# TCLResearchEurope/ptdeco

Measured on AMD Instinct MI355X. Metric: layers decomposed/sec (incl. covariance+SVD), higher is better.
Workload: dtype f64

## Files before the change

### ptdeco_amd/csrc/eigh_tridiag.hip

```cpp
#include <algorithm>
#include <atomic>
#include <cmath>
#include <cstdlib>
#include <cstring>
#include <functional>
#include <mutex>
#include <vector>

#include <hip/hip_ext.h>

#include "common.h"
#include "kernels.h"

namespace ptd {

int gemm_f64(const double* A, int64_t sam, int64_t sak, const double* B, int64_t sbk, int64_t sbn, double* C,
             int64_t ldc, int64_t M, int64_t N, int64_t K, double alpha, bool beta1, int ksplit, hipStream_t st);
int gemm_f64_pair(const double* A, const double* B, const double* A2, const double* B2, int64_t sam, int64_t sak,
                  int64_t sbk, int64_t sbn, double* C, int64_t ldc, int64_t M, int64_t N, int64_t K, double alpha,
                  double* row0_out, hipStream_t st, int batch = 1, int64_t bstride_elems = 0);
int gemm_f64_slabs(const double* A, int64_t sam, int64_t sak, const double* B, int64_t sbk, int64_t sbn, double* C,
                   int64_t ldc, int64_t slab, int64_t M, int64_t N, int64_t K, double alpha, int ksplit, int* nslabs,
                   bool lower_only, hipStream_t st);

// ... 146 lines not shown
        cs->alpha = colbuf[j + 1] - delta * vprev[j + 1];
      }
    }
  }
}

constexpr int TR = 64, TC = 256, TQ = TC / TR;

struct SymPart {
  double* rowpart;
  double* colpart;
  int64_t ldp;
  int nI;
  int enabled;
};

__device__ __forceinline__ double transpose_reduce16(double (&p)[16], int lane) {
  {
    const bool hi = lane & 32;
#pragma unroll
    for (int t = 0; t < 8; ++t) {
      const double send = hi ? p[t] : p[t + 8];
      const double keep = hi ? p[t + 8] : p[t];
      p[t] = keep + __shfl_xor(send, 32);
    }
  }
  {
    const bool hi = lane & 16;
#pragma unroll
    for (int t = 0; t < 4; ++t) {
      const double send = hi ? p[t] : p[t + 4];
      const double keep = hi ? p[t + 4] : p[t];
      p[t] = keep + __shfl_xor(send, 16);
    }
  }
  {
    const bool hi = lane & 8;
#pragma unroll
    for (int t = 0; t < 2; ++t) {
      const double send = hi ? p[t] : p[t + 2];
      const double keep = hi ? p[t + 2] : p[t];
      p[t] = keep + __shfl_xor(send, 8);
    }
  }
  {
    const bool hi = lane & 4;
    const double send = hi ? p[0] : p[1];
    const double keep = hi ? p[1] : p[0];
    p[0] = keep + __shfl_xor(send, 4);
  }
  p[0] += __shfl_xor(p[0], 2);
  p[0] += __shfl_xor(p[0], 1);
  return p[0];
}

template <bool GEN>
__device__ __forceinline__ void symv2_tile_body(const double2 (&a0)[16], const double2 (&a1)[16], const double2 xa,
                                                const double2 xb, const double* __restrict__ xs, int rbase, int nclamp,
                                                int cA, int cB, double (&p)[16], double (&acc)[4]) {
#pragma unroll
  for (int t = 0; t < 16; ++t) {
    const double xr = xs[t];
    double r0 = a0[t].x, r1 = a0[t].y, r2 = a1[t].x, r3 = a1[t].y;
    double c0 = r0, c1 = r1, c2 = r2, c3 = r3;
    if (GEN) {
      const int R = min(rbase + t, nclamp);
      r0 = (cA <= R) ? r0 : 0.0;     c0 = (cA < R) ? c0 : 0.0;
      r1 = (cA + 1 <= R) ? r1 : 0.0; c1 = (cA + 1 < R) ? c1 : 0.0;
      r2 = (cB <= R) ? r2 : 0.0;     c2 = (cB < R) ? c2 : 0.0;
      r3 = (cB + 1 <= R) ? r3 : 0.0; c3 = (cB + 1 < R) ? c3 : 0.0;
    }
    p[t] = (r0 * xa.x + r1 * xa.y) + (r2 * xb.x + r3 * xb.y);
    acc[0] += c0 * xr; acc[1] += c1 * xr; acc[2] += c2 * xr; acc[3] += c3 * xr;
  }
}

#ifdef PTD_RES_PROF
__device__ int symv_dbg;
extern "C" void ptd_debug_symv(int v) { (void)hipMemcpyToSymbol(HIP_SYMBOL(symv_dbg), &v, sizeof(int)); }
#define SYMV_DBG(BIT) (symv_dbg & (BIT))
#else
#define SYMV_DBG(BIT) false
#endif
__global__ __launch_bounds__(256) void sytrd_symv2_kernel(const double* __restrict__ A, int64_t ld, int n, int j, int i,
                                                          const double* __restrict__ colbuf,
                                                          const double* __restrict__ Vp,
                                                          const double* __restrict__ Wp, int64_t ldv,
                                                          const double* __restrict__ wraw_prev,
                                                          const double* __restrict__ partial2, int nparts2,
                                                          const double* __restrict__ taus, SymPart sp, int ntiles,
                                                          int nextra, double* __restrict__ qv,
                                                          double* __restrict__ cb, double* __restrict__ px2,
                                                          ColState* __restrict__ cs, size_t bstride) {
  const size_t boff_ = (size_t)blockIdx.y * bstride;
  PTD_BATCH(A); PTD_BATCH(colbuf); PTD_BATCH(Vp); PTD_BATCH(Wp); PTD_BATCH(wraw_prev); PTD_BATCH(partial2);
  PTD_BATCH(taus); PTD_BATCH(sp.rowpart); PTD_BATCH(sp.colpart); PTD_BATCH(qv); PTD_BATCH(cb); PTD_BATCH(px2);
  PTD_BATCH(cs);
  __shared__ __attribute__((aligned(16))) double xs[TR];
  __shared__ __attribute__((aligned(16))) double colred[4][TC];
  __shared__ double part[4][SROWS];
  const int tid = threadIdx.x, lane = tid & 63, wid = tid >> 6;
  const int b = blockIdx.x;
  const double* vprev = Vp + (int64_t)max(i - 1, 0) * ldv;
  if (SYMV_DBG(1)) return;
  if (b < ntiles) {
    const int g0 = (j + 1) / TC;
    int u = (int)((sqrtf(2.f * (float)b + 1.f) - 1.f) * 0.5f);
    while (TQ / 2 * u * (u + 1) > b) --u;
    while (TQ / 2 * (u + 1) * (u + 2) <= b) ++u;
    const int rem = b - TQ / 2 * u * (u + 1);
    const int I = TQ * (g0 + u) + rem / (u + 1), J = g0 + rem % (u + 1);
    const int R0 = I * TR, C0 = J * TC;
    if (R0 + TR - 1 < j + 1 || R0 >= n) return;
    const int cA = C0 + 2 * lane, cB = cA + 128;
    const int rbase = R0 + 16 * wid;
    double2 a0[16], a1[16];
    const bool liveA = (C0 + 127 >= j + 1) && (C0 <= R0 + TR - 1) && (cA + 1 >= j + 1);
    const bool liveB = (C0 + 255 >= j + 1) && (C0 + 128 <= R0 + TR - 1) && (cB + 1 >= j + 1);
    if (C0 + TC - 1 > R0) {
#pragma unroll
      for (int t = 0; t < 16; ++t) {
        const int rr = min(rbase + t, n - 1);
        const double* rowp = A + (int64_t)rr * ld;
        a0[t] = (liveA && cA <= rr) ? *reinterpret_cast<const double2*>(rowp + cA) : double2{0.0, 0.0};
        a1[t] = (liveB && cB <= rr) ? *reinterpret_cast<const double2*>(rowp + cB) : double2{0.0, 0.0};
      }
    } else {
#pragma unroll
      for (int t = 0; t < 16; ++t) {
        const double* rowp = A + (int64_t)min(rbase + t, n - 1) * ld;
        a0[t] = liveA ? *reinterpret_cast<const double2*>(rowp + cA) : double2{0.0, 0.0};
        a1[t] = liveB ? *reinterpret_cast<const double2*>(rowp + cB) : double2{0.0, 0.0};
      }
    }
    if (SYMV_DBG(2)) {
      double sink = 0.0;
#pragma unroll
      for (int t = 0; t < 16; ++t) sink += a0[t].x + a0[t].y + a1[t].x + a1[t].y;
      if (sink == 1.2345e-300) xs[0] = sink;
      return;
    }
    double2 xa = *reinterpret_cast<const double2*>(colbuf + cA);
    double2 xb = *reinterpret_cast<const double2*>(colbuf + cB);
    const double2 va = *reinterpret_cast<const double2*>(vprev + cA);
    const double2 vb = *reinterpret_cast<const double2*>(vprev + cB);
    double xrow = 0.0, vrow = 0.0;
    const int Rx = R0 + tid;
    const bool rowok = tid < TR && Rx >= j + 2 && Rx < n;
    if (rowok) { xrow = colbuf[Rx]; vrow = vprev[Rx]; }
    double delta = 0.0;
    if (i > 0) delta = -taus[j - 1] * wave_total(partial2, nparts2, lane);
    if (tid < TR) xs[tid] = rowok ? xrow - delta * vrow : 0.0;
    xa.x = (cA >= j + 2) ? xa.x - delta * va.x : 0.0;
    xa.y = (cA + 1 >= j + 2) ? xa.y - delta * va.y : 0.0;
    xb.x = (cB >= j + 2) ? xb.x - delta * vb.x : 0.0;
    xb.y = (cB + 1 >= j + 2) ? xb.y - delta * vb.y : 0.0;
    __syncthreads();
    double p[16], acc[4] = {0.0, 0.0, 0.0, 0.0};
    const bool general = (C0 + TC - 1 > R0) || (C0 + TC > n);
    if (general) symv2_tile_body<true>(a0, a1, xa, xb, xs + 16 * wid, rbase, n - 1, cA, cB, p, acc);
    else symv2_tile_body<false>(a0, a1, xa, xb, xs + 16 * wid, rbase, n - 1, cA, cB, p, acc);
    const double rowsum = transpose_reduce16(p, lane);
    if ((lane & 3) == 0) sp.rowpart[(int64_t)J * sp.ldp + rbase + (lane >> 2)] = rowsum;
    *reinterpret_cast<double2*>(&colred[wid][2 * lane]) = double2{acc[0], acc[1]};
    *reinterpret_cast<double2*>(&colred[wid][128 + 2 * lane]) = double2{acc[2], acc[3]};
    __syncthreads();
    sp.colpart[(int64_t)I * sp.ldp + C0 + tid] =
        (colred[0][tid] + colred[1][tid]) + (colred[2][tid] + colred[3][tid]);
    return;
  }
  double delta = 0.0;
  if (i > 0) delta = -taus[j - 1] * wave_total(partial2, nparts2, lane);
  if (b < ntiles + nextra) {
    const int total = 2 * i;
    const int g0 = (b - ntiles) * SROWS;
    const double* rp[SROWS];
    double acc[SROWS];
#pragma unroll
    for (int t = 0; t < SROWS; ++t) {
      const int g = min(g0 + t, total - 1);
      if (g < i) rp[t] = (g == i - 1) ? wraw_prev : Wp + (int64_t)g * ldv;
      else rp[t] = Vp + (int64_t)(g - i) * ldv;
      acc[t] = 0.0;
    }
    const int cstart = (j + 2) & ~1;
    for (int c = cstart + 2 * lane + 128 * wid; c < n; c += 512) {
      double2 xa = *reinterpret_cast<const double2*>(colbuf + c);
      const double2 va = *reinterpret_cast<const double2*>(vprev + c);
      xa.x -= delta * va.x; xa.y -= delta * va.y;
      if (c < j + 2) xa.x = 0.0;
      if (c + 1 >= n) xa.y = 0.0;
#pragma unroll
      for (int t = 0; t < SROWS; ++t) {
        const double2 r2 = *reinterpret_cast<const double2*>(rp[t] + c);
        acc[t] += r2.x * xa.x + r2.y * xa.y;
      }
    }
#pragma unroll
    for (int t = 0; t < SROWS; ++t) {
      const double sdot = wave_sum_d(acc[t]);
      if (lane == 0) part[wid][t] = sdot;
    }
    __syncthreads();
    if (tid < SROWS && g0 + tid < total) {
      const int g = g0 + tid;
      const double sdot = (part[0][tid] + part[1][tid]) + (part[2][tid] + part[3][tid]);
      if (g < i) {
        const double* row = (g == i - 1) ? wraw_prev : Wp + (int64_t)g * ldv;
        cb[g] = sdot;
        cb[NB + g] = row[j + 1];
      } else {
        const int k = g - i;
        cb[2 * NB + k] = sdot;
        cb[3 * NB + k] = Vp[(int64_t)k * ldv + j + 1];
      }
    }
    return;
  }
  {
    const int chunk = b - ntiles - nextra;
    const int r = j + 1 + chunk * 256 + tid;
    double x2 = 0.0;
    if (r < n) {
      qv[r] = A[(int64_t)r * ld + j + 1];
      if (r >= j + 2) {
        const double xr = colbuf[r] - delta * vprev[r];
        x2 = xr * xr;
      }
    }
    x2 = wave_sum_d(x2);
    if (lane == 0) part[wid][0] = x2;
    __syncthreads();
    if (tid == 0) {
      px2[chunk] = (part[0][0] + part[1][0]) + (part[2][0] + part[3][0]);
      if (chunk == 0) {
        cs->delta = delta;
        cs->alpha = colbuf[j + 1] - delta * vprev[j + 1];
      }
    }
  }
}

__global__ __launch_bounds__(256) void sytrd_alpha_kernel(const double* __restrict__ A, int64_t ld, int n, int jn,
                                                          int in, int do_next, double* __restrict__ Vp,
                                                          double* __restrict__ Wp, int64_t ldv,
                                                          const double* __restrict__ wraw_prev,
                                                          double* __restrict__ wraw_cur,
                                                          double* __restrict__ colbuf, const double* __restrict__ sd,
                                                          const double* __restrict__ qv,
                                                          const double* __restrict__ cb,
                                                          const double* __restrict__ px2, int npx2,
                                                          const ColState* __restrict__ cs,
                                                          double* __restrict__ partial2, double* __restrict__ d,
                                                          double* __restrict__ e, double* __restrict__ taus,
                                                          SymPart sp, size_t bstride) {
  const size_t boff_ = (size_t)blockIdx.y * bstride;
  PTD_BATCH(A); PTD_BATCH(Vp); PTD_BATCH(Wp); PTD_BATCH(wraw_prev); PTD_BATCH(wraw_cur); PTD_BATCH(colbuf);
  PTD_BATCH(sd); PTD_BATCH(qv); PTD_BATCH(cb); PTD_BATCH(px2); PTD_BATCH(cs); PTD_BATCH(partial2); PTD_BATCH(d);
  PTD_BATCH(e); PTD_BATCH(taus); PTD_BATCH(sp.rowpart); PTD_BATCH(sp.colpart);
  __shared__ double c1[NB], c2[NB], wj1[NB], vj1[NB];
  __shared__ double part1[4][64], part2[4][64];
  __shared__ double vs[64], wfs[64];
  __shared__ double red[4], red2[4];
  __shared__ double sdp[4][64];
  __shared__ double wrj_s;
  const int tid = threadIdx.x, lane = tid & 63, wid = tid >> 6;
  const int j = jn - 1, i = in - 1;
  const int r = jn + blockIdx.x * 64 + lane;
  double px = 0.0;
  for (int q = tid; q < npx2; q += 256) px += px2[q];
  const double delta = cs->delta, alpha = cs->alpha;
  double r_sdW = 0.0, r_qW = 0.0, r_sdV = 0.0, r_qV = 0.0, r_vj1 = 0.0, r_wj1 = 0.0, r_vpjn = 0.0;
  if (tid < i) {
    r_sdW = cb[tid]; r_qW = cb[NB + tid]; r_sdV = cb[2 * NB + tid]; r_qV = cb[3 * NB + tid];
    r_vj1 = Vp[(int64_t)tid * ldv + jn];
    r_wj1 = (tid == i - 1) ? wraw_prev[jn] : Wp[(int64_t)tid * ldv + jn];
    if (tid == i - 1) r_vpjn = Vp[(int64_t)(i - 1) * ldv + jn];
  }
  double r_col = 0.0, r_vprev = 0.0, r_wprev = 0.0, r_qv = 0.0, r_a = 0.0;
  if (wid == 0 && r < n) {
    r_col = colbuf[r];
    if (i > 0) { r_vprev = Vp[(int64_t)(i - 1) * ldv + r]; r_wprev = wraw_prev[r]; }
    r_qv = qv[r];
    if (do_next) r_a = A[(int64_t)jn * ld + r];
  }
  double pv[NB / 4], pw[NB / 4];
#pragma unroll
  for (int q = 0; q < NB / 4; ++q) {
    const int k = wid + 4 * q;
    pv[q] = 0.0; pw[q] = 0.0;
    if (k < i && r < n) {
      pv[q] = Vp[(int64_t)k * ldv + r];
      if (k < i - 1) pw[q] = Wp[(int64_t)k * ldv + r];
    }
  }
  double sdacc = 0.0, sdjn = 0.0;
  if (sp.enabled) {
    const int J0 = jn / TC;
    if (r < n) {
      const int nrow = r / TC - J0 + 1, i0 = r / TR, cnt = nrow + sp.nI - i0;
      constexpr int SDU = 20;
      for (int k0 = wid; k0 < cnt; k0 += 4 * SDU) {
        double v[SDU];
#pragma unroll
        for (int q = 0; q < SDU; ++q) {
          const int k = k0 + 4 * q;
          v[q] = 0.0;
          if (k < cnt)
            v[q] = (k < nrow) ? sp.rowpart[(int64_t)(J0 + k) * sp.ldp + r]
                              : sp.colpart[(int64_t)(i0 + k - nrow) * sp.ldp + r];
        }
        double s4[SDU / 4];
#pragma unroll
        for (int q = 0; q < SDU / 4; ++q) s4[q] = (v[4 * q] + v[4 * q + 1]) + (v[4 * q + 2] + v[4 * q + 3]);
        sdacc += ((s4[0] + s4[1]) + (s4[2] + s4[3])) + s4[4];
      }
    }
    const int i0 = jn / TR, cnt = 1 + sp.nI - i0;
    for (int k = tid; k < cnt; k += 256)
      sdjn += (k == 0) ? sp.rowpart[(int64_t)J0 * sp.ldp + jn] : sp.colpart[(int64_t)(i0 + k - 1) * sp.ldp + jn];
  } else {
    if (wid == 0 && r < n) sdacc = sd[r];
// ... 1882 lines not shown
struct TridiagPlan {
  int n;
  int64_t ld;
  int npanels;
  size_t off_A, off_V, off_W, off_col, off_p, off_part, off_refl, off_d, off_e, off_e2, off_ds, off_tau, off_bounds, off_lam;
  size_t off_u1, off_u2, off_u3, off_lm, off_sw, off_G, off_T, off_W1, off_W2, off_wraw, off_wraw2, off_part2, off_cbuf;
  size_t off_qv, off_px2, off_rowpart, off_colpart, off_gpart, off_tall, off_res, off_twd, off_twe, off_twl;
  int64_t ldp;
  size_t total;
};

TridiagPlan tridiag_plan(int64_t n) {
  TridiagPlan p{};
  p.n = (int)n;
  p.ld = (int64_t)align_up((size_t)n, n >= 512 ? TC : 8);
  if (n >= 512) {
    const char* pad = getenv("PTD_LD_PAD");
    p.ld += pad ? atoi(pad) / 2 * 2 : 64;
  }
  p.ldp = (int64_t)align_up((size_t)n, TC);
  p.npanels = (int)ceil_div(n, NB);
  size_t o = 0;
  auto take = [&](size_t bytes) { size_t at = o; o += align_up(bytes, 256); return at; };
  p.off_A = take((size_t)p.npanels * NB * p.ld * 8);
  p.off_V = take((size_t)p.npanels * NB * p.ld * 8);
  p.off_W = take((size_t)NB * p.ld * 8);
  p.off_col = take((size_t)(p.ldp + 8) * 8);
  p.off_p = take((size_t)(n + 8) * 8);
  p.off_part = take((size_t)(ceil_div(n, 64) + 8) * 8);
  p.off_refl = take(256);
  p.off_d = take((size_t)n * 8);
  p.off_e = take((size_t)n * 8);
  p.off_e2 = take((size_t)n * 8);
  p.off_ds = take((size_t)n * 8);
  p.off_tau = take((size_t)n * 8);
  p.off_bounds = take(64);
  p.off_lam = take((size_t)n * 8);
  p.off_u1 = take((size_t)n * n * 8);
  p.off_u2 = take((size_t)n * n * 8);
  p.off_u3 = take((size_t)n * n * 8);
  p.off_lm = take((size_t)n * n * 8);
  p.off_sw = take((size_t)n * n);
  p.off_G = take((size_t)NB * NB * 8);
  p.off_T = take((size_t)NB * NB * 8);
  p.off_W1 = take((size_t)NB * n * 8);
  p.off_W2 = take((size_t)NB * n * 8);
  p.off_wraw = take((size_t)(n + 8) * 8);
  p.off_wraw2 = take((size_t)(n + 8) * 8);
  p.off_part2 = take((size_t)(ceil_div(n, 64) + 8) * 8);
  p.off_cbuf = take((size_t)4 * NB * 8);
  p.off_qv = take((size_t)(n + 8) * 8);
  p.off_px2 = take((size_t)(ceil_div(n + 2 * NB, SROWS) + 8) * 8);
  p.off_rowpart = take((size_t)ceil_div(n, TC) * p.ldp * 8);
  p.off_colpart = take((size_t)ceil_div(n, TR) * p.ldp * 8);
  p.off_gpart = take((size_t)p.npanels * ceil_div(n, GCH) * NB * NB * 8);
  p.off_tall = take((size_t)p.npanels * NB * NB * 8);
  p.off_res = take(8192 + 4 * (size_t)RES_XS * 8);
  p.off_twd = take((size_t)TW_MAXN * 8);
  p.off_twe = take((size_t)TW_MAXN * 8);
  p.off_twl = take((size_t)(n + 16) * 4);
  p.total = o;
  return p;
}

struct SymvTimer {
  std::vector<hipEvent_t> ev;
  int stride = 1;
  int limit = INT32_MAX;
  bool sampled(int j) const { return j < limit && j % stride == stride / 2; }
  hipEvent_t start(int j) const { return ev[2 * (size_t)(j / stride)]; }
  hipEvent_t stop(int j) const { return ev[2 * (size_t)(j / stride) + 1]; }
};

constexpr int MAX_DEVICES = 64;
struct DeviceState {
  std::once_flag probed;
  int cus = 0;
  bool gfx950 = false;
  bool occupancy_ok = false;
  std::atomic<int> chains{1};
  std::atomic<int> inflight{0};
  std::atomic<int> skip{0};
  std::atomic<int> failures{0};
};
DeviceState g_dev[MAX_DEVICES];

DeviceState& device_state() {
  int dev = 0;
  (void)hipGetDevice(&dev);
  return g_dev[(dev < 0 || dev >= MAX_DEVICES) ? 0 : dev];
}

void probe_device(DeviceState& ds) {
  int dev = 0;
  (void)hipGetDevice(&dev);
  hipDeviceProp_t prop;
  if (hipGetDeviceProperties(&prop, dev) != hipSuccess) return;
  ds.cus = prop.multiProcessorCount;
  ds.gfx950 = strncmp(prop.gcnArchName, "gfx950", 6) == 0;
  const void* kernels[7] = {reinterpret_cast<const void*>(sytrd_resident_kernel<RES_WG, RES_MAX, false>),
                            reinterpret_cast<const void*>(sytrd_resident_kernel<RES_WG, RES_MID, false>),
                            reinterpret_cast<const void*>(sytrd_resident_kernel<RESG_WG, RESG_MAX, true>),
                            reinterpret_cast<const void*>(sytrd_resident3_kernel),
                            reinterpret_cast<const void*>(sytrd_resident4_kernel<R4_MAX>),
                            reinterpret_cast<const void*>(sytrd_resident4_kernel<R4B_MAX>),
                            reinterpret_cast<const void*>(sytrd_resident4_kernel<R4C_MAX>)};
  bool ok = true;
  for (const void* f : kernels) {
    int blocks = 0;
    const int threads = (f == kernels[4] || f == kernels[5] || f == kernels[6]) ? R4_T : RES_T;
    ok = ok && hipFuncSetAttribute(f, hipFuncAttributeMaxDynamicSharedMemorySize, (int)RES_LDS) == hipSuccess &&
         hipOccupancyMaxActiveBlocksPerMultiprocessor(&blocks, f, threads, RES_LDS) == hipSuccess && blocks >= 1;
  }
  ds.occupancy_ok = ok;
}

int resident_mode() {
  const char* env = getenv("PTD_SYTRD_RESIDENT");
  return env ? atoi(env) : 7;
}
int resident_start(int n) {
  const int mode = resident_mode();
  if (mode == 0 || n < 128) return n;
  DeviceState& ds = device_state();
  std::call_once(ds.probed, probe_device, std::ref(ds));
  const char* fake = getenv("PTD_SYTRD_FAKE_CUS");
  const int cus = fake ? atoi(fake) : ds.cus;
  if (cus != RESG_WG || !ds.gfx950 || !ds.occupancy_ok) return n;
  if (ds.chains.load(std::memory_order_relaxed) > 1 || ds.inflight.load(std::memory_order_relaxed) > 1) return n;
  int left = ds.skip.load(std::memory_order_relaxed);
  while (left > 0)
    if (ds.skip.compare_exchange_weak(left, left - 1, std::memory_order_relaxed)) return n;
  const int cap = n <= RES_MAX ? RES_MAX : (mode >= 7 ? R4C_MAX : (mode == 6 ? R4B_MAX : (mode == 5 ? R4_MAX : (mode == 4 ? R3_MAX : (mode == 3 ? RESG_MAX : RES_MAX)))));
  return n <= cap ? 0 : (int)align_up((size_t)(n - cap), NB);
}
void resident_failed(int status) {
  if (status == 3) return;
  DeviceState& ds = device_state();
  const int f = std::min(ds.failures.fetch_add(1) + 1, 14);
  ds.skip.store(32 << f, std::memory_order_relaxed);
}
struct InflightGuard {
  DeviceState& ds;
  InflightGuard() : ds(device_state()) { ds.inflight.fetch_add(1); }
  ~InflightGuard() { ds.inflight.fetch_sub(1); }
};

template <typename T>
static inline T* batch_host(T* p, size_t off) { return reinterpret_cast<T*>(reinterpret_cast<char*>(p) + off); }

int* resident_status(const TridiagPlan& p, char* base) { return &reinterpret_cast<ResCtl*>(base + p.off_res)->fail; }

int sytrd_f64(const TridiagPlan& p, char* base, SymvTimer* timer, bool resident, hipStream_t st, int count = 1,
              size_t bstride = 0) {
  const int n = p.n;
  const unsigned nb = (unsigned)std::max(count, 1);
  if (nb > 1) resident = false;
  if (nb == 1) bstride = 0;
  const int64_t ld = p.ld;
  double* Aw = reinterpret_cast<double*>(base + p.off_A);
  double* Vall = reinterpret_cast<double*>(base + p.off_V);
  double* Wp = reinterpret_cast<double*>(base + p.off_W);
  double* colbuf = reinterpret_cast<double*>(base + p.off_col);
  double* pbuf = reinterpret_cast<double*>(base + p.off_p);
  double* d = reinterpret_cast<double*>(base + p.off_d);
  double* e = reinterpret_cast<double*>(base + p.off_e);
  double* taus = reinterpret_cast<double*>(base + p.off_tau);

  double* wr[2] = {reinterpret_cast<double*>(base + p.off_wraw), reinterpret_cast<double*>(base + p.off_wraw2)};
  double* partial2 = reinterpret_cast<double*>(base + p.off_part2);
  double* cbuf = reinterpret_cast<double*>(base + p.off_cbuf);
  double* sd = pbuf;
  double* qv = reinterpret_cast<double*>(base + p.off_qv);
  double* px2 = reinterpret_cast<double*>(base + p.off_px2);
  ColState* cs = reinterpret_cast<ColState*>(base + p.off_refl);
  SymPart sp{reinterpret_cast<double*>(base + p.off_rowpart), reinterpret_cast<double*>(base + p.off_colpart), p.ldp,
             (int)ceil_div(n, TR), 0};
  const char* symv_env = getenv("PTD_SYMV");
  const char* symv_min_env = getenv("PTD_SYMV_MIN");
  const int sym_min = (symv_env && !strcmp(symv_env, "full")) ? INT32_MAX
                      : std::max(512, symv_min_env ? atoi(symv_min_env) : 1024);
  bool prev_sym = false;
  for (unsigned b = 0; b < nb; ++b) {
    const size_t bo = b * bstride;
    PTD_CHECK_HIP(hipMemsetAsync(batch_host(Vall, bo), 0, (size_t)p.npanels * NB * ld * 8, st));
    PTD_CHECK_HIP(hipMemsetAsync(batch_host(taus, bo), 0, (size_t)n * 8, st));
    PTD_CHECK_HIP(hipMemsetAsync(batch_host(e, bo), 0, (size_t)n * 8, st));
    PTD_CHECK_HIP(hipMemsetAsync(batch_host(colbuf, bo), 0, (size_t)(p.ldp + 8) * 8, st));
    PTD_CHECK_HIP(hipMemsetAsync(batch_host(Wp, bo), 0, (size_t)NB * ld * 8, st));
    PTD_CHECK_HIP(hipMemsetAsync(batch_host(wr[0], bo), 0, (size_t)(n + 8) * 8, st));
    PTD_CHECK_HIP(hipMemsetAsync(batch_host(wr[1], bo), 0, (size_t)(n + 8) * 8, st));
  }
  bool colbuf_ready = false;
  const int t_res = resident ? resident_start(n) : n;
  if (timer) timer->limit = t_res;
  ResCtl* rctl = reinterpret_cast<ResCtl*>(base + p.off_res);
  for (unsigned b = 0; b < nb; ++b) PTD_CHECK_HIP(hipMemsetAsync(batch_host(rctl, b * bstride), 0, sizeof(ResCtl), st));
  for (int pn = 0; pn < p.npanels; ++pn) {
    const int j0 = pn * NB;
    if (j0 == t_res && n - j0 >= 2) {
      double* X = reinterpret_cast<double*>(base + p.off_res + 8192);
      const bool attr =
          hipFuncSetAttribute(reinterpret_cast<const void*>(sytrd_resident_kernel<RES_WG, RES_MAX, false>),
                              hipFuncAttributeMaxDynamicSharedMemorySize, (int)RES_LDS) == hipSuccess &&
          hipFuncSetAttribute(reinterpret_cast<const void*>(sytrd_resident_kernel<RES_WG, RES_MID, false>),
                              hipFuncAttributeMaxDynamicSharedMemorySize, (int)RES_LDS) == hipSuccess &&
          hipFuncSetAttribute(reinterpret_cast<const void*>(sytrd_resident_kernel<RESG_WG, RESG_MAX, true>),
                              hipFuncAttributeMaxDynamicSharedMemorySize, (int)RES_LDS) == hipSuccess &&
          hipFuncSetAttribute(reinterpret_cast<const void*>(sytrd_resident3_kernel),
                              hipFuncAttributeMaxDynamicSharedMemorySize, (int)RES_LDS) == hipSuccess &&
          hipFuncSetAttribute(reinterpret_cast<const void*>(sytrd_resident4_kernel<R4_MAX>),
                              hipFuncAttributeMaxDynamicSharedMemorySize, (int)RES_LDS) == hipSuccess &&
          hipFuncSetAttribute(reinterpret_cast<const void*>(sytrd_resident4_kernel<R4B_MAX>),
                              hipFuncAttributeMaxDynamicSharedMemorySize, (int)RES_LDS) == hipSuccess &&
          hipFuncSetAttribute(reinterpret_cast<const void*>(sytrd_resident4_kernel<R4C_MAX>),
                              hipFuncAttributeMaxDynamicSharedMemorySize, (int)RES_LDS) == hipSuccess;
      PTD_REQUIRE(attr, "sytrd_f64: cannot reserve the LDS of the resident tail");
      static std::atomic<unsigned long long> calls{0};
      static_assert(RESG_MAX < (1 << 16), "sequence numbers of one launch: epoch .. epoch + m");
      int t1 = j0, t2 = j0, t3 = j0, t4 = j0, t5 = j0;
      if (n - j0 > R4B_MAX) {
        const unsigned long long epoch = (calls.fetch_add(1) + 1) << 16;
        t5 = n - R4B_MAX;
        hipLaunchKernelGGL((sytrd_resident4_kernel<R4C_MAX>), dim3(RESG_WG), dim3(R4_T), RES_LDS, st, Aw, ld, n, j0,
                           t5 - j0, Vall, taus, d, e, rctl, X, epoch);
      }
      t4 = t5;
      if (n - t5 > R4_MAX) {
        const unsigned long long epoch = (calls.fetch_add(1) + 1) << 16;
        t4 = n - R4_MAX;
        hipLaunchKernelGGL((sytrd_resident4_kernel<R4B_MAX>), dim3(RESG_WG), dim3(R4_T), RES_LDS, st, Aw, ld, n, t5,
                           t4 - t5, Vall, taus, d, e, rctl, X, epoch);
      }
      t3 = t4;
      if (n - t4 > R3_MAX) {
        const unsigned long long epoch = (calls.fetch_add(1) + 1) << 16;
        t3 = n - R3_MAX;
        hipLaunchKernelGGL((sytrd_resident4_kernel<R4_MAX>), dim3(RESG_WG), dim3(R4_T), RES_LDS, st, Aw, ld, n, t4,
                           t3 - t4, Vall, taus, d, e, rctl, X, epoch);
      }
      t2 = t3;
      if (n - t3 > RESG_MAX) {
        const unsigned long long epoch = (calls.fetch_add(1) + 1) << 16;
        t2 = n - RESG_MAX;
        hipLaunchKernelGGL(sytrd_resident3_kernel, dim3(RESG_WG), dim3(RES_T), RES_LDS, st, Aw, ld, n, t3, t2 - t3, Vall,
                           taus, d, e, rctl, X, epoch);
      }
      const int one_xcd = resident_mode() == 1 ? RES_MAX : RES_MID;
      if (n - t2 > one_xcd) {
        const unsigned long long epoch = (calls.fetch_add(1) + 1) << 16;
        t1 = n - one_xcd;
        hipLaunchKernelGGL((sytrd_resident_kernel<RESG_WG, RESG_MAX, true>), dim3(RESG_WG), dim3(RES_T), RES_LDS, st, Aw, ld,
                           n, t2, t1 - t2, Vall, taus, d, e, rctl, X, epoch);
      }
      if (n - t1 > RES_MAX) {
        const unsigned long long epoch = (calls.fetch_add(1) + 1) << 16;
        const int t15 = n - RES_MAX;
        hipLaunchKernelGGL((sytrd_resident_kernel<RES_WG, RES_MID, false>), dim3(8 * RES_WG), dim3(RES_T), RES_LDS, st, Aw,
                           ld, n, t1, t15 - t1, Vall, taus, d, e, rctl, X, epoch);
        PTD_CHECK_HIP(hipMemsetAsync(&rctl->reg, 0, sizeof(unsigned), st));
        t1 = t15;
      }
      const unsigned long long epoch = (calls.fetch_add(1) + 1) << 16;
      hipLaunchKernelGGL((sytrd_resident_kernel<RES_WG, RES_MAX, false>), dim3(8 * RES_WG), dim3(RES_T), RES_LDS, st, Aw, ld,
                         n, t1, n - t1 - 1, Vall, taus, d, e, rctl, X, epoch);
      if (resident_mode() == 2)
        PTD_CHECK_HIP(hipMemsetAsync(&rctl->fail, 3, 1, st));
      break;
    }
    const int cols = std::min(NB, n - j0);
    double* Vp = Vall + (size_t)pn * NB * ld;
    int nparts2 = 0, npx2 = 0;
    bool open = false;
    for (int i = 0; i < cols; ++i) {
      const int j = j0 + i;
      if (i == 0) {
        if (!colbuf_ready)
          hipLaunchKernelGGL(sytrd_colinit_kernel, dim3((unsigned)ceil_div(n - j, 256), nb), dim3(256), 0, st, Aw, ld, n,
                             j, colbuf, bstride);
        colbuf_ready = false;
      } else {
        const int blocks = (int)ceil_div(n - j, 64);
        SymPart spa = sp;
        spa.enabled = prev_sym;
        hipLaunchKernelGGL(sytrd_alpha_kernel, dim3(blocks, nb), dim3(256), 0, st, Aw, ld, n, j, i, 1, Vp, Wp, ld,
                           wr[(i & 1)], wr[(i - 1) & 1], colbuf, sd, qv, cbuf, px2, npx2, cs, partial2, d, e, taus,
                           spa, bstride);
        nparts2 = blocks;
      }
      const int m = n - j - 1;
      if (m >= sym_min && n >= 512) {
        const int U = (int)ceil_div(n, TC) - (j + 1) / TC;
        const int ntiles = TQ / 2 * U * (U + 1);
        const int nextra = (int)ceil_div(2 * i, SROWS);
        npx2 = (int)ceil_div(m, 256);
        const dim3 grid((unsigned)(ntiles + nextra + npx2), nb);
        const bool timed = timer && timer->sampled(j);
        hipEvent_t ev0 = timed ? timer->start(j) : nullptr, ev1 = timed ? timer->stop(j) : nullptr;
        hipExtLaunchKernelGGL(sytrd_symv2_kernel, grid, dim3(256), 0, st, ev0, ev1, 0, Aw, ld, n, j, i, colbuf, Vp, Wp,
                              ld, wr[(i + 1) & 1], partial2, nparts2, taus, sp, ntiles, nextra, qv, cbuf, px2, cs, bstride);
        prev_sym = true;
        open = true;
      } else if (m > 0) {
        prev_sym = false;
        const int rows = m + 2 * i;
        npx2 = (int)ceil_div(rows, SROWS);
        if (timer && timer->sampled(j)) {
          hipExtLaunchKernelGGL(sytrd_symv_kernel, dim3(npx2, nb), dim3(256), 0, st, timer->start(j),
                                timer->stop(j), 0, Aw, ld, n, j, i, colbuf, Vp, Wp, ld,
                                wr[(i + 1) & 1], partial2, nparts2, taus, sd, qv, cbuf, px2, cs, bstride);
        } else {
          hipLaunchKernelGGL(sytrd_symv_kernel, dim3(npx2, nb), dim3(256), 0, st, Aw, ld, n, j, i, colbuf, Vp, Wp, ld,
                             wr[(i + 1) & 1], partial2, nparts2, taus, sd, qv, cbuf, px2, cs, bstride);
        }
        open = true;
      } else {
        hipLaunchKernelGGL(sytrd_last_kernel, dim3(1, nb), dim3(64), 0, st, n, i, colbuf, partial2, nparts2, taus, d, bstride);
        open = false;
      }
    }
    const int t0 = j0 + cols;
    if (open) {
      const int blocks = (int)ceil_div(n - t0, 64);
      SymPart spa = sp;
      spa.enabled = prev_sym;
      hipLaunchKernelGGL(sytrd_alpha_kernel, dim3(std::max(blocks, 1), nb), dim3(256), 0, st, Aw, ld, n, t0, cols, 0, Vp,
                         Wp, ld, wr[(cols & 1)], wr[(cols - 1) & 1], colbuf, sd, qv, cbuf, px2, npx2, cs, partial2,
                         d, e, taus, spa, bstride);
      const int mt = n - t0;
      if (mt > 0) {
        hipLaunchKernelGGL(sytrd_wfix_kernel, dim3((unsigned)ceil_div(mt, 256), nb), dim3(256), 0, st, n, t0, cols - 1,
                           t0 - 1, Vp, Wp, ld, wr[(cols - 1) & 1], partial2, std::max(blocks, 1), taus, bstride);
        double* At = Aw + (int64_t)t0 * ld + t0;
        const int rc = gemm_f64_pair(Vp + t0, Wp + t0, Wp + t0, Vp + t0, 1, ld, ld, 1, At, ld, mt, mt, cols, -1.0,
                                     colbuf + t0, st, (int)nb, (int64_t)(bstride / 8));
        colbuf_ready = true;
        if (rc != PTD_OK) return rc;
      }
    }
  }
  PTD_CHECK_LAUNCH("sytrd_f64");
  return PTD_OK;
}

int tridiag_eigenvalues(const TridiagPlan& p, char* base, int first, hipStream_t st) {
  const int n = p.n;
  double* d = reinterpret_cast<double*>(base + p.off_d);
  double* e = reinterpret_cast<double*>(base + p.off_e);
  double* e2 = reinterpret_cast<double*>(base + p.off_e2);
  double* bounds = reinterpret_cast<double*>(base + p.off_bounds);
  double* lam = reinterpret_cast<double*>(base + p.off_lam);
  double* ds = reinterpret_cast<double*>(base + p.off_ds);
  hipLaunchKernelGGL(tridiag_bounds_kernel, dim3(1), dim3(1024), 0, st, d, e, n, bounds);
  hipLaunchKernelGGL(scale_tridiag_kernel, dim3((unsigned)ceil_div(n, 256)), dim3(256), 0, st, d, e, n, bounds, ds, e2);
  if (first > 0) PTD_CHECK_HIP(hipMemsetAsync(lam, 0xFF, (size_t)first * 8, st));
  if (n <= 4096)
    hipLaunchKernelGGL((tridiag_bisect_kernel<true>), dim3((unsigned)ceil_div(n - first, 4)), dim3(256), (size_t)n * 16, st,
                       ds, e2, n, bounds, lam, first);
  else
    hipLaunchKernelGGL((tridiag_bisect_kernel<false>), dim3((unsigned)ceil_div(n - first, 4)), dim3(256), 0, st, ds, e2,
                       n, bounds, lam, first);
  PTD_CHECK_LAUNCH("tridiag_eigenvalues");
  return PTD_OK;
}


namespace {
__global__ void sum_slabs_kernel(double* __restrict__ out, const double* __restrict__ S, int64_t total, int ns) {
  for (int64_t i = blockIdx.x * (int64_t)blockDim.x + threadIdx.x; i < total; i += (int64_t)gridDim.x * blockDim.x) {
    double acc = S[i];
    for (int q = 1; q < ns; ++q) acc += S[(int64_t)q * total + i];
    out[i] = acc;
  }
}

__global__ void gram_pad_kernel(double* __restrict__ G, int mp, int nvec) {
  for (int64_t e = blockIdx.x * (int64_t)blockDim.x + threadIdx.x; e < (int64_t)mp * mp; e += (int64_t)gridDim.x * blockDim.x) {
    const int r = (int)(e / mp), c = (int)(e % mp);
    if (r >= nvec || c >= nvec) G[e] = r == c ? 1.0 : 0.0;
  }
}
}

// ... 491 lines not shown
```

Baseline: 18.01.

## Add persistent double-buffered SYMV kernel and alternate tile order per column

```diff
diff --git a/ptdeco_amd/csrc/eigh_tridiag.hip b/ptdeco_amd/csrc/eigh_tridiag.hip
--- a/ptdeco_amd/csrc/eigh_tridiag.hip
+++ b/ptdeco_amd/csrc/eigh_tridiag.hip
@@ -252,6 +252,16 @@
 #else
 #define SYMV_DBG(BIT) false
 #endif
+__device__ __forceinline__ void symv2_tile_ij(int b, int j, int& I, int& J) {
+  const int g0 = (j + 1) / TC;
+  int u = (int)((sqrtf(2.f * (float)b + 1.f) - 1.f) * 0.5f);
+  while (TQ / 2 * u * (u + 1) > b) --u;
+  while (TQ / 2 * (u + 1) * (u + 2) <= b) ++u;
+  const int rem = b - TQ / 2 * u * (u + 1);
+  I = TQ * (g0 + u) + rem / (u + 1);
+  J = g0 + rem % (u + 1);
+}
+
 __global__ __launch_bounds__(256) void sytrd_symv2_kernel(const double* __restrict__ A, int64_t ld, int n, int j, int i,
                                                           const double* __restrict__ colbuf,
                                                           const double* __restrict__ Vp,
@@ -261,8 +271,8 @@
                                                           const double* __restrict__ taus, SymPart sp, int ntiles,
                                                           int nextra, double* __restrict__ qv,
                                                           double* __restrict__ cb, double* __restrict__ px2,
-                                                          ColState* __restrict__ cs, size_t bstride) {
-  const size_t boff_ = (size_t)blockIdx.y * bstride;
+                                                          ColState* __restrict__ cs, size_t bstride, int rev) {
+  const size_t boff_ = (size_t)(rev ? gridDim.y - 1 - blockIdx.y : blockIdx.y) * bstride;
   PTD_BATCH(A); PTD_BATCH(colbuf); PTD_BATCH(Vp); PTD_BATCH(Wp); PTD_BATCH(wraw_prev); PTD_BATCH(partial2);
   PTD_BATCH(taus); PTD_BATCH(sp.rowpart); PTD_BATCH(sp.colpart); PTD_BATCH(qv); PTD_BATCH(cb); PTD_BATCH(px2);
   PTD_BATCH(cs);
@@ -270,16 +280,12 @@
   __shared__ __attribute__((aligned(16))) double colred[4][TC];
   __shared__ double part[4][SROWS];
   const int tid = threadIdx.x, lane = tid & 63, wid = tid >> 6;
-  const int b = blockIdx.x;
+  const int b = (rev && (int)blockIdx.x < ntiles) ? ntiles - 1 - (int)blockIdx.x : (int)blockIdx.x;
   const double* vprev = Vp + (int64_t)max(i - 1, 0) * ldv;
   if (SYMV_DBG(1)) return;
   if (b < ntiles) {
-    const int g0 = (j + 1) / TC;
-    int u = (int)((sqrtf(2.f * (float)b + 1.f) - 1.f) * 0.5f);
-    while (TQ / 2 * u * (u + 1) > b) --u;
-    while (TQ / 2 * (u + 1) * (u + 2) <= b) ++u;
-    const int rem = b - TQ / 2 * u * (u + 1);
-    const int I = TQ * (g0 + u) + rem / (u + 1), J = g0 + rem % (u + 1);
+    int I, J;
+    symv2_tile_ij(b, j, I, J);
     const int R0 = I * TR, C0 = J * TC;
     if (R0 + TR - 1 < j + 1 || R0 >= n) return;
     const int cA = C0 + 2 * lane, cB = cA + 128;
@@ -408,6 +414,261 @@
         cs->alpha = colbuf[j + 1] - delta * vprev[j + 1];
       }
     }
+  }
+}
+
+constexpr int SYMV_MAXB = 16;
+
+constexpr int SYMV_OOB = 0x7ffffff0;
+typedef double native_double2 __attribute__((ext_vector_type(2)));
+typedef __attribute__((address_space(1))) const native_double2 gconst_double2;
+typedef __attribute__((address_space(1))) const double gconst_double;
+__device__ __forceinline__ double2 gload2(const double* p) {
+  const native_double2 v = *(gconst_double2*)p;
+  return double2{v.x, v.y};
+}
+__device__ __forceinline__ double gload(const double* p) { return *(gconst_double*)p; }
+__device__ __forceinline__ void gstore(double* p, double v) { *(__attribute__((address_space(1))) double*)p = v; }
+__device__ __forceinline__ double2 bload2(__amdgpu_buffer_rsrc_t r, int off) {
+  const native_double2 v = __builtin_bit_cast(native_double2, __builtin_amdgcn_raw_buffer_load_b128(r, off, 0, 0));
+  return double2{v.x, v.y};
+}
+
+struct Symv2Tile {
+  int mat, R0, C0, I, J;
+  bool live;
+};
+
+__device__ __forceinline__ Symv2Tile symv2_tile(int u, int count, int n, int j) {
+  Symv2Tile t{0, 0, 0, 0, 0, false};
+  if (u < 0) return t;
+  t.mat = u % count;
+  symv2_tile_ij(u / count, j, t.I, t.J);
+  t.R0 = t.I * TR;
+  t.C0 = t.J * TC;
+  t.live = !(t.R0 + TR - 1 < j + 1 || t.R0 >= n);
+  if (!t.live) { t.R0 = 0; t.C0 = 0; }
+  return t;
+}
+
+struct Symv2X {
+  double2 xa, xb, va, vb;
+  double xrow, vrow;
+};
+
+template <int H>
+__device__ __forceinline__ void symv2_load_half(double2 (&a)[8][2], __amdgpu_buffer_rsrc_t rA, int64_t ld, int n, int j,
+                                                const Symv2Tile& t, int lane, int wid) {
+  const int cA = t.C0 + 2 * lane, cB = cA + 128, rbase = t.R0 + 16 * wid;
+  const bool liveA = t.live && (t.C0 + 127 >= j + 1) && (t.C0 <= t.R0 + TR - 1) && (cA + 1 >= j + 1);
+  const bool liveB = t.live && (t.C0 + 255 >= j + 1) && (t.C0 + 128 <= t.R0 + TR - 1) && (cB + 1 >= j + 1);
+#pragma unroll
+  for (int q = 0; q < 8; ++q) {
+    const int rr = min(rbase + 8 * H + q, n - 1);
+    const int row = (int)((int64_t)rr * ld * 8);
+    a[q][0] = bload2(rA, (liveA && cA <= rr) ? row + 8 * cA : SYMV_OOB);
+    a[q][1] = bload2(rA, (liveB && cB <= rr) ? row + 8 * cB : SYMV_OOB);
+  }
+}
+
+__device__ __forceinline__ void symv2_load_x(Symv2X& x, const double* __restrict__ colbuf,
+                                             const double* __restrict__ vprev, int n, const Symv2Tile& t, int tid,
+                                             int lane) {
+  const int cA = t.C0 + 2 * lane, cB = cA + 128;
+  const int Rx = min(t.R0 + tid, n - 1);
+  x.xa = gload2(colbuf + cA);
+  x.xb = gload2(colbuf + cB);
+  x.va = gload2(vprev + cA);
+  x.vb = gload2(vprev + cB);
+  x.xrow = gload(colbuf + Rx);
+  x.vrow = gload(vprev + Rx);
+}
+
+template <bool GEN, int H>
+__device__ __forceinline__ void symv2_half_body(const double2 (&a)[8][2], const double2 xa, const double2 xb,
+                                                const double* __restrict__ xs, int rbase, int nclamp, int cA, int cB,
+                                                double (&p)[16], double (&acc)[4]) {
+#pragma unroll
+  for (int q = 0; q < 8; ++q) {
+    const int t = 8 * H + q;
+    const double xr = xs[t];
+    double r0 = a[q][0].x, r1 = a[q][0].y, r2 = a[q][1].x, r3 = a[q][1].y;
+    double c0 = r0, c1 = r1, c2 = r2, c3 = r3;
+    if (GEN) {
+      const int R = min(rbase + t, nclamp);
+      r0 = (cA <= R) ? r0 : 0.0;     c0 = (cA < R) ? c0 : 0.0;
+      r1 = (cA + 1 <= R) ? r1 : 0.0; c1 = (cA + 1 < R) ? c1 : 0.0;
+      r2 = (cB <= R) ? r2 : 0.0;     c2 = (cB < R) ? c2 : 0.0;
+      r3 = (cB + 1 <= R) ? r3 : 0.0; c3 = (cB + 1 < R) ? c3 : 0.0;
+    }
+    p[t] = (r0 * xa.x + r1 * xa.y) + (r2 * xb.x + r3 * xb.y);
+    acc[0] += c0 * xr; acc[1] += c1 * xr; acc[2] += c2 * xr; acc[3] += c3 * xr;
+  }
+}
+
+__global__ __launch_bounds__(256, 2) void sytrd_symv2_persistent_kernel(const double* __restrict__ A, int64_t ld, int n, int j,
+                                                             int i, const double* __restrict__ colbuf,
+                                                             const double* __restrict__ Vp,
+                                                             const double* __restrict__ Wp, int64_t ldv,
+                                                             const double* __restrict__ wraw_prev,
+                                                             const double* __restrict__ partial2, int nparts2,
+                                                             const double* __restrict__ taus, SymPart sp, int ntiles,
+                                                             int nextra, int nchunks, int count,
+                                                             double* __restrict__ qv, double* __restrict__ cb,
+                                                             double* __restrict__ px2, ColState* __restrict__ cs,
+                                                             size_t bstride) {
+  __shared__ __attribute__((aligned(16))) double xs[TR];
+  __shared__ __attribute__((aligned(16))) double colred[4][TC];
+  __shared__ double part[4][SROWS];
+  __shared__ double dls[SYMV_MAXB];
+  const int tid = threadIdx.x, lane = tid & 63, wid = tid >> 6;
+  const int G = gridDim.x;
+  const int nt = ntiles * count;
+  const int nunits = nt + count * (nextra + nchunks);
+  const int64_t vprev_off = (int64_t)max(i - 1, 0) * ldv;
+  for (int m = wid; m < count; m += 4) {
+    double dl = 0.0;
+    if (i > 0) {
+      const size_t boff_ = (size_t)m * bstride;
+      dl = -batch_ptr(taus, boff_)[j - 1] * wave_total(batch_ptr(partial2, boff_), nparts2, lane);
+    }
+    if (lane == 0) dls[m] = dl;
+  }
+  __syncthreads();
+
+  const uint32_t abytes = (uint32_t)((int64_t)n * ld * 8);
+  auto rsrc_A = [&](int m) {
+    return __builtin_amdgcn_make_buffer_rsrc((void*)batch_ptr(A, (size_t)m * bstride), (short)0, (int)abytes,
+                                             0x00020000);
+  };
+  auto load_x = [&](Symv2X& x, const Symv2Tile& t) {
+    const size_t off = (size_t)t.mat * bstride;
+    symv2_load_x(x, batch_ptr(colbuf, off), batch_ptr(Vp, off) + vprev_off, n, t, tid, lane);
+  };
+  int u = blockIdx.x;
+  double2 h0[8][2], h1[8][2];
+  Symv2Tile ct = symv2_tile(u < nt ? u : -1, count, n, j);
+  Symv2X cx;
+  load_x(cx, ct);
+  symv2_load_half<0>(h0, rsrc_A(ct.mat), ld, n, j, ct, lane, wid);
+  while (u < nt) {
+    const size_t boff_ = (size_t)ct.mat * bstride;
+    const int cA = ct.C0 + 2 * lane, cB = cA + 128, rbase = ct.R0 + 16 * wid;
+    const bool general = (ct.C0 + TC - 1 > ct.R0) || (ct.C0 + TC > n);
+    symv2_load_half<1>(h1, rsrc_A(ct.mat), ld, n, j, ct, lane, wid);
+    double p[16], acc[4] = {0.0, 0.0, 0.0, 0.0};
+    double2 xa = cx.xa, xb = cx.xb;
+    if (ct.live) {
+      const double delta = dls[ct.mat];
+      const int Rx = ct.R0 + tid;
+      if (tid < TR) xs[tid] = (Rx >= j + 2 && Rx < n) ? cx.xrow - delta * cx.vrow : 0.0;
+      xa.x = (cA >= j + 2) ? xa.x - delta * cx.va.x : 0.0;
+      xa.y = (cA + 1 >= j + 2) ? xa.y - delta * cx.va.y : 0.0;
+      xb.x = (cB >= j + 2) ? xb.x - delta * cx.vb.x : 0.0;
+      xb.y = (cB + 1 >= j + 2) ? xb.y - delta * cx.vb.y : 0.0;
+      __syncthreads();
+      if (general) symv2_half_body<true, 0>(h0, xa, xb, xs + 16 * wid, rbase, n - 1, cA, cB, p, acc);
+      else symv2_half_body<false, 0>(h0, xa, xb, xs + 16 * wid, rbase, n - 1, cA, cB, p, acc);
+    }
+    const int un = u + G;
+    const Symv2Tile nxt = symv2_tile(un < nt ? un : -1, count, n, j);
+    load_x(cx, nxt);
+    symv2_load_half<0>(h0, rsrc_A(nxt.mat), ld, n, j, nxt, lane, wid);
+    if (ct.live) {
+      if (general) symv2_half_body<true, 1>(h1, xa, xb, xs + 16 * wid, rbase, n - 1, cA, cB, p, acc);
+      else symv2_half_body<false, 1>(h1, xa, xb, xs + 16 * wid, rbase, n - 1, cA, cB, p, acc);
+      const double rowsum = transpose_reduce16(p, lane);
+      if ((lane & 3) == 0) gstore(batch_ptr(sp.rowpart, boff_) + (int64_t)ct.J * sp.ldp + rbase + (lane >> 2), rowsum);
+      *reinterpret_cast<double2*>(&colred[wid][2 * lane]) = double2{acc[0], acc[1]};
+      *reinterpret_cast<double2*>(&colred[wid][128 + 2 * lane]) = double2{acc[2], acc[3]};
+      __syncthreads();
+      gstore(batch_ptr(sp.colpart, boff_) + (int64_t)ct.I * sp.ldp + ct.C0 + tid,
+             (colred[0][tid] + colred[1][tid]) + (colred[2][tid] + colred[3][tid]));
+    }
+    u = un;
+    ct = nxt;
+  }
+
+  for (; u < nunits; u += G) {
+    const int v = u - nt, per = nextra + nchunks;
+    const int m = v / per, b = v % per;
+    const size_t boff_ = (size_t)m * bstride;
+    const double* Am = batch_ptr(A, boff_);
+    const double* colm = batch_ptr(colbuf, boff_);
+    const double* Vm = batch_ptr(Vp, boff_);
+    const double* Wm = batch_ptr(Wp, boff_);
+    const double* wrm = batch_ptr(wraw_prev, boff_);
+    const double* vprev = Vm + vprev_off;
+    const double delta = dls[m];
+    if (b < nextra) {
+      const int total = 2 * i;
+      const int g0 = b * SROWS;
+      const double* rp[SROWS];
+      double acc[SROWS];
+#pragma unroll
+      for (int t = 0; t < SROWS; ++t) {
+        const int g = min(g0 + t, total - 1);
+        if (g < i) rp[t] = (g == i - 1) ? wrm : Wm + (int64_t)g * ldv;
+        else rp[t] = Vm + (int64_t)(g - i) * ldv;
+        acc[t] = 0.0;
+      }
+      const int cstart = (j + 2) & ~1;
+      for (int c = cstart + 2 * lane + 128 * wid; c < n; c += 512) {
+        double2 xa = *reinterpret_cast<const double2*>(colm + c);
+        const double2 va = *reinterpret_cast<const double2*>(vprev + c);
+        xa.x -= delta * va.x; xa.y -= delta * va.y;
+        if (c < j + 2) xa.x = 0.0;
+        if (c + 1 >= n) xa.y = 0.0;
+#pragma unroll
+        for (int t = 0; t < SROWS; ++t) {
+          const double2 r2 = *reinterpret_cast<const double2*>(rp[t] + c);
+          acc[t] += r2.x * xa.x + r2.y * xa.y;
+        }
+      }
+#pragma unroll
+      for (int t = 0; t < SROWS; ++t) {
+        const double sdot = wave_sum_d(acc[t]);
+        if (lane == 0) part[wid][t] = sdot;
+      }
+      __syncthreads();
+      if (tid < SROWS && g0 + tid < total) {
+        const int g = g0 + tid;
+        const double sdot = (part[0][tid] + part[1][tid]) + (part[2][tid] + part[3][tid]);
+        double* cbm = batch_ptr(cb, boff_);
+        if (g < i) {
+          const double* row = (g == i - 1) ? wrm : Wm + (int64_t)g * ldv;
+          cbm[g] = sdot;
+          cbm[NB + g] = row[j + 1];
+        } else {
+          const int k = g - i;
+          cbm[2 * NB + k] = sdot;
+          cbm[3 * NB + k] = Vm[(int64_t)k * ldv + j + 1];
+        }
+      }
+    } else {
+      const int chunk = b - nextra;
+      const int r = j + 1 + chunk * 256 + tid;
+      double x2 = 0.0;
+      if (r < n) {
+        batch_ptr(qv, boff_)[r] = Am[(int64_t)r * ld + j + 1];
+        if (r >= j + 2) {
+          const double xr = colm[r] - delta * vprev[r];
+          x2 = xr * xr;
+        }
+      }
+      x2 = wave_sum_d(x2);
+      if (lane == 0) part[wid][0] = x2;
+      __syncthreads();
+      if (tid == 0) {
+        batch_ptr(px2, boff_)[chunk] = (part[0][0] + part[1][0]) + (part[2][0] + part[3][0]);
+        if (chunk == 0) {
+          ColState* csm = batch_ptr(cs, boff_);
+          csm->delta = delta;
+          csm->alpha = colm[j + 1] - delta * vprev[j + 1];
+        }
+      }
+    }
+    __syncthreads();
   }
 }
 
@@ -2456,6 +2717,9 @@
   std::atomic<int> inflight{0};
   std::atomic<int> skip{0};
   std::atomic<int> failures{0};
+  std::once_flag symv_probed;
+  int symv_cus = 0;
+  int symv_per_cu = 0;
 };
 DeviceState g_dev[MAX_DEVICES];
 
@@ -2520,6 +2784,23 @@
   ~InflightGuard() { ds.inflight.fetch_sub(1); }
 };
 
+int symv_persistent_slots() {
+  DeviceState& ds = device_state();
+  std::call_once(ds.symv_probed, [&ds]() {
+    int dev = 0, cus = 0, per_cu = 0;
+    (void)hipGetDevice(&dev);
+    if (hipDeviceGetAttribute(&cus, hipDeviceAttributeMultiprocessorCount, dev) == hipSuccess &&
+        hipOccupancyMaxActiveBlocksPerMultiprocessor(&per_cu, reinterpret_cast<const void*>(sytrd_symv2_persistent_kernel),
+                                                     256, 0) == hipSuccess && cus > 0 && per_cu > 0) {
+      ds.symv_cus = cus;
+      ds.symv_per_cu = per_cu;
+    }
+  });
+  const char* env = getenv("PTD_SYMV_WG_PER_CU");
+  const int per_cu = env ? std::min(std::max(atoi(env), 1), ds.symv_per_cu) : ds.symv_per_cu;
+  return ds.symv_cus * per_cu;
+}
+
 template <typename T>
 static inline T* batch_host(T* p, size_t off) { return reinterpret_cast<T*>(reinterpret_cast<char*>(p) + off); }
 
@@ -2555,6 +2836,13 @@
   const int sym_min = (symv_env && !strcmp(symv_env, "full")) ? INT32_MAX
                       : std::max(512, symv_min_env ? atoi(symv_min_env) : 1024);
   bool prev_sym = false;
+  const char* alt_env = getenv("PTD_SYMV_ALTERNATE");
+  const bool alternate = !(alt_env && !strcmp(alt_env, "0"));
+  int symv_slots = 0;
+  if (symv_env && !strcmp(symv_env, "persistent") && (int)nb <= SYMV_MAXB && (int64_t)n * ld * 8 < SYMV_OOB) {
+    symv_slots = symv_persistent_slots();
+    PTD_REQUIRE(symv_slots > 0, "sytrd_f64: occupancy query of sytrd_symv2_persistent_kernel failed");
+  }
   for (unsigned b = 0; b < nb; ++b) {
     const size_t bo = b * bstride;
     PTD_CHECK_HIP(hipMemsetAsync(batch_host(Vall, bo), 0, (size_t)p.npanels * NB * ld * 8, st));
@@ -2668,11 +2956,18 @@
         const int ntiles = TQ / 2 * U * (U + 1);
         const int nextra = (int)ceil_div(2 * i, SROWS);
         npx2 = (int)ceil_div(m, 256);
-        const dim3 grid((unsigned)(ntiles + nextra + npx2), nb);
         const bool timed = timer && timer->sampled(j);
         hipEvent_t ev0 = timed ? timer->start(j) : nullptr, ev1 = timed ? timer->stop(j) : nullptr;
-        hipExtLaunchKernelGGL(sytrd_symv2_kernel, grid, dim3(256), 0, st, ev0, ev1, 0, Aw, ld, n, j, i, colbuf, Vp, Wp,
-                              ld, wr[(i + 1) & 1], partial2, nparts2, taus, sp, ntiles, nextra, qv, cbuf, px2, cs, bstride);
+        if (symv_slots > 0) {
+          const int units = (int)nb * (ntiles + nextra + npx2);
+          hipExtLaunchKernelGGL(sytrd_symv2_persistent_kernel, dim3((unsigned)std::min(units, symv_slots)), dim3(256), 0,
+                                st, ev0, ev1, 0, Aw, ld, n, j, i, colbuf, Vp, Wp, ld, wr[(i + 1) & 1], partial2, nparts2,
+                                taus, sp, ntiles, nextra, npx2, (int)nb, qv, cbuf, px2, cs, bstride);
+        } else {
+          hipExtLaunchKernelGGL(sytrd_symv2_kernel, dim3((unsigned)(ntiles + nextra + npx2), nb), dim3(256), 0, st,
+                                ev0, ev1, 0, Aw, ld, n, j, i, colbuf, Vp, Wp, ld, wr[(i + 1) & 1], partial2, nparts2,
+                                taus, sp, ntiles, nextra, qv, cbuf, px2, cs, bstride, alternate ? (j & 1) : 0);
+        }
         prev_sym = true;
         open = true;
       } else if (m > 0) {
```

Result: no change. 18.03, median of 6 (+0.1%).
